# microsoft/esvit

Hardware: NVIDIA H100
Metric: multi-crop images/sec, Swin-T W7 pretrain step (2 global 224^2 + 8 local 96^2 crops, DDINOLoss V+R, K=65536) (higher is better)
Workload: dtype bf16

## Files before the change

### esvit_b200/csrc/window_attn.cu

```cuda
#include <cstdlib>

#include "wa_common.cuh"
#include "window_attn7.cuh"
#include "window_attn14.cuh"
#include "window_attn_probs.cuh"

namespace wa {

static bool make_geo(Geo& g, int B, int H, int W, int C, int nH, int ws, int shift) {
  if (B <= 0 || C != nH * HD || (ws != 7 && ws != 14) || shift < 0 || shift >= ws) return false;
  g.B = B; g.H = H; g.W = W; g.C = C; g.nH = nH; g.shift = shift;
  g.Hp = (H + ws - 1) / ws * ws;
  g.Wp = (W + ws - 1) / ws * ws;
  g.nWy = g.Hp / ws;
  g.nWx = g.Wp / ws;
  const char* d = getenv("ESVIT_ATTN_DBG");
  g.dbg = d ? atoi(d) : 0;
  return true;
}

static int windows_grid(int nwin, int nH, int per_sm) {
  int gy = esvit_num_sms() * per_sm / nH;
  if (gy < 1) gy = 1;
  const char* e = getenv("ESVIT_ATTN_GY");
  if (e && atoi(e) > 0) gy = atoi(e);
  return gy > nwin ? nwin : gy;
}

template <typename K>
static cudaError_t opt_in_smem(K kernel, size_t smem) {
  return smem > 48 * 1024 ? cudaFuncSetAttribute(kernel, cudaFuncAttributeMaxDynamicSharedMemorySize, (int)smem)
                          : cudaSuccess;
}

}

ESVIT_API int esvit_window_attn_expand_bias(const float* bias_table, float* bias_ws, int nH, int ws, void* stream) {
  if (nH <= 0 || (ws != 7 && ws != 14) || !bias_table) return ESVIT_ERR_BAD_ARG;
  if (ws == 7) {
    if (!bias_ws) return ESVIT_ERR_BAD_ARG;
    wa::expand_bias7_kernel<<<nH, 256, 0, (cudaStream_t)stream>>>(bias_table, bias_ws, nH);
  }
  ESVIT_LAUNCH_CHECK();
}

ESVIT_API int esvit_window_attn_fwd(const void* qkv, const void* qkv_bias, const float* bias_table, float* bias_ws,
                                    int bias_ready, void* out, float* lse, int B, int H, int W, int C, int nH, int ws,
                                    int shift, float scale, void* stream) {
  wa::Geo g;
  if (!wa::make_geo(g, B, H, W, C, nH, ws, shift)) return ESVIT_ERR_BAD_ARG;
  const int nwin = B * g.nWy * g.nWx;
  cudaStream_t st = (cudaStream_t)stream;
  const bf16* q = (const bf16*)qkv;
  const bf16* qb = (const bf16*)qkv_bias;
  if (ws == 7) {
    if (!bias_ws) return ESVIT_ERR_BAD_ARG;
    if (!bias_ready) wa::expand_bias7_kernel<<<nH, 256, 0, st>>>(bias_table, bias_ws, nH);
    const size_t smem = wa::fwd7_smem();
    const int gx = wa::windows_grid(nwin, nH, 16);
    if (shift > 0)
      wa::window_attn_fwd7_kernel<true><<<dim3(nH, gx), 128, smem, st>>>(q, qb, bias_ws, (bf16*)out, lse, g, scale, nwin);
    else
      wa::window_attn_fwd7_kernel<false><<<dim3(nH, gx), 128, smem, st>>>(q, qb, bias_ws, (bf16*)out, lse, g, scale, nwin);
  } else {
    const size_t smem = wa::fwd14_smem();
    cudaError_t e = wa::opt_in_smem(wa::window_attn_fwd14_kernel<true>, smem);
    if (e == cudaSuccess) e = wa::opt_in_smem(wa::window_attn_fwd14_kernel<false>, smem);
    if (e != cudaSuccess) return (int)e;
    const dim3 grid(nH, wa::windows_grid(nwin, nH, 2));
    if (shift > 0)
      wa::window_attn_fwd14_kernel<true><<<grid, wa::T14, smem, st>>>(q, qb, bias_table, (bf16*)out, lse, g, scale, nwin);
    else
      wa::window_attn_fwd14_kernel<false><<<grid, wa::T14, smem, st>>>(q, qb, bias_table, (bf16*)out, lse, g, scale, nwin);
  }
  ESVIT_LAUNCH_CHECK();
}

ESVIT_API int esvit_window_attn_bwd(const void* qkv, const void* qkv_bias, const float* bias_table, float* bias_ws,
                                    int bias_ready, const void* out, const void* dout, const float* lse, void* dqkv,
                                    float* dbias_table, float* dqkv_bias, int B, int H, int W, int C, int nH, int ws,
                                    int shift, float scale, void* stream) {
  wa::Geo g;
  if (!wa::make_geo(g, B, H, W, C, nH, ws, shift)) return ESVIT_ERR_BAD_ARG;
  const int nwin = B * g.nWy * g.nWx;
  cudaStream_t st = (cudaStream_t)stream;
  const bf16* q = (const bf16*)qkv;
  const bf16* qb = (const bf16*)qkv_bias;
  if (ws == 7) {
    if (!bias_ws) return ESVIT_ERR_BAD_ARG;
    if (!bias_ready) wa::expand_bias7_kernel<<<nH, 256, 0, st>>>(bias_table, bias_ws, nH);
    const size_t smem = wa::bwd7_smem();
    cudaError_t e = wa::opt_in_smem(wa::window_attn_bwd7_kernel<true>, smem);
    if (e == cudaSuccess) e = wa::opt_in_smem(wa::window_attn_bwd7_kernel<false>, smem);
    if (e != cudaSuccess) return (int)e;
    const int gx = wa::windows_grid(nwin, nH, 12);
    if (shift > 0)
      wa::window_attn_bwd7_kernel<true><<<dim3(nH, gx), 128, smem, st>>>(q, qb, bias_ws, (const bf16*)out,
                                                                         (const bf16*)dout, lse, (bf16*)dqkv,
                                                                         dbias_table, dqkv_bias, g, scale, nwin);
    else
      wa::window_attn_bwd7_kernel<false><<<dim3(nH, gx), 128, smem, st>>>(q, qb, bias_ws, (const bf16*)out,
                                                                          (const bf16*)dout, lse, (bf16*)dqkv,
                                                                          dbias_table, dqkv_bias, g, scale, nwin);
  } else {
    if (!bias_ws) return ESVIT_ERR_BAD_ARG;
    const size_t smem = wa::bwd14_smem();
    cudaError_t e = wa::opt_in_smem(wa::window_attn_bwd14_kernel<true>, smem);
    if (e == cudaSuccess) e = wa::opt_in_smem(wa::window_attn_bwd14_kernel<false>, smem);
    if (e == cudaSuccess) e = cudaMemsetAsync(bias_ws, 0, (size_t)nH * wa::GACC14 * sizeof(float), st);
    if (e != cudaSuccess) return (int)e;
    const dim3 grid(nH, wa::windows_grid(nwin, nH, 2));
    if (shift > 0)
      wa::window_attn_bwd14_kernel<true><<<grid, wa::T14, smem, st>>>(q, qb, bias_table, (const bf16*)out, (const bf16*)dout,
                                                                      lse, (bf16*)dqkv, bias_ws, dqkv_bias, g, scale, nwin);
    else
      wa::window_attn_bwd14_kernel<false><<<grid, wa::T14, smem, st>>>(q, qb, bias_table, (const bf16*)out, (const bf16*)dout,
                                                                       lse, (bf16*)dqkv, bias_ws, dqkv_bias, g, scale, nwin);
    wa::fold_dbias14_kernel<<<dim3(27, nH), 192, 0, st>>>(bias_ws, dbias_table, nH);
  }
  ESVIT_LAUNCH_CHECK();
}

ESVIT_API int esvit_window_attn_probs(const void* qkv, const void* qkv_bias, const float* bias_table, float* bias_ws,
                                      int bias_ready, float* probs, int B, int H, int W, int C, int nH, int ws,
                                      int shift, float scale, void* stream) {
  wa::Geo g;
  if (!wa::make_geo(g, B, H, W, C, nH, ws, shift) || !qkv || !qkv_bias || !bias_table || !probs) return ESVIT_ERR_BAD_ARG;
  const int nwin = B * g.nWy * g.nWx;
  cudaStream_t st = (cudaStream_t)stream;
  const bf16* q = (const bf16*)qkv;
  const bf16* qb = (const bf16*)qkv_bias;
  if (ws == 7) {
    if (!bias_ws) return ESVIT_ERR_BAD_ARG;
    if (!bias_ready) wa::expand_bias7_kernel<<<nH, 256, 0, st>>>(bias_table, bias_ws, nH);
    const size_t smem = wa::probs7_smem();
    const dim3 grid(nH, wa::windows_grid(nwin, nH, 16));
    if (shift > 0)
      wa::window_attn_probs7_kernel<true><<<grid, 128, smem, st>>>(q, qb, bias_ws, probs, g, scale, nwin);
    else
      wa::window_attn_probs7_kernel<false><<<grid, 128, smem, st>>>(q, qb, bias_ws, probs, g, scale, nwin);
  } else {
    const size_t smem = wa::probs14_smem();
    cudaError_t e = wa::opt_in_smem(wa::window_attn_probs14_kernel<true>, smem);
    if (e == cudaSuccess) e = wa::opt_in_smem(wa::window_attn_probs14_kernel<false>, smem);
    if (e != cudaSuccess) return (int)e;
    const dim3 grid(nH, wa::windows_grid(nwin, nH, 2));
    if (shift > 0)
      wa::window_attn_probs14_kernel<true><<<grid, wa::T14, smem, st>>>(q, qb, bias_table, probs, g, scale, nwin);
    else
      wa::window_attn_probs14_kernel<false><<<grid, wa::T14, smem, st>>>(q, qb, bias_table, probs, g, scale, nwin);
  }
  ESVIT_LAUNCH_CHECK();
}
```

### esvit_b200/csrc/window_attn7.cuh

```cuda
#pragma once
#include "wa_common.cuh"

namespace wa {

constexpr int BLD = 72;
constexpr int TILE7 = 64 * LD;

__global__ void __launch_bounds__(256) expand_bias7_kernel(const float* __restrict__ bias_table, float* __restrict__ bexp,
                                                           int nH) {
  const int h = blockIdx.x;
  for (int i = threadIdx.x; i < 64 * 64; i += blockDim.x) {
    const int row = i >> 6, col = i & 63;
    float v = -INFINITY;
    if (col < 49) v = row < 49 ? bias_table[bias_index<7>(row, col) * nH + h] * LOG2E : 0.f;
    bexp[(long long)h * 4096 + i] = v;
  }
}

template <bool BWD, int NTHREADS = 128, int NPART = 3>
__device__ __forceinline__ void issue7(const Geo& g, int win, int h, const bf16* __restrict__ qkv,
                                       const uint4 (&bchunk)[3], const bf16* __restrict__ dout,
                                       const bf16* __restrict__ out, const float* __restrict__ lse, bf16* tiles,
                                       float* Lraw, int* tok, int* rid) {
  constexpr int WS = 7, NT = 49;
  const int wx = win % g.nWx, wy = (win / g.nWx) % g.nWy, b = win / (g.nWx * g.nWy);
  const int c16 = threadIdx.x & 3;
#pragma unroll
  for (int kk = 0; kk < 256 / NTHREADS; kk++) {
    const int t = (threadIdx.x >> 2) + (NTHREADS / 4) * kk;
    int tk = -1, r = 0;
    if (t < NT) slot_info<WS>(g, b, wy, wx, t, tk, r);
    const bf16* src_row = qkv + (long long)(tk >= 0 ? tk : 0) * 3 * g.C + h * HD + c16 * 8;
    const int nbytes = (t < NT && g.dbg != 1) ? 16 : 0;
    if (t < NT && tk < 0) {
#pragma unroll
      for (int part = 0; part < NPART; part++)
        *reinterpret_cast<uint4*>(tiles + part * TILE7 + t * LD + c16 * 8) = bchunk[part];
    } else {
#pragma unroll
      for (int part = 0; part < NPART; part++)
        cp_async16(tiles + part * TILE7 + t * LD + c16 * 8, src_row + part * g.C, nbytes);
    }
    if (BWD) {
      const long long off = (long long)(tk >= 0 ? tk : 0) * g.C + h * HD + c16 * 8;
      const int nb = (tk >= 0 && g.dbg != 1) ? 16 : 0;
      cp_async16(tiles + 3 * TILE7 + t * LD + c16 * 8, dout + off, nb);
      cp_async16(tiles + 4 * TILE7 + t * LD + c16 * 8, out + off, nb);
    }
    if (c16 == 0) {
      tok[t] = tk;
      rid[t] = r;
      if (BWD) cp_async4(Lraw + t, lse + ((long long)win * g.nH + h) * NT + (t < NT ? t : 0), t < NT ? 4 : 0);
    }
  }
}

template <bool SHIFT>
__global__ void __launch_bounds__(128, 4) window_attn_fwd7_kernel(
    const bf16* __restrict__ qkv, const bf16* __restrict__ qkv_bias, const float* __restrict__ bexp,
    bf16* __restrict__ out, float* __restrict__ lse, Geo g, float scale, int nwin_total) {
  constexpr int WS = 7;
  using C = Cfg<WS>;
  static_assert(C::KP == 64 && C::NW == 4, "fast path assumes a 64-slot window and 4 warps");
  extern __shared__ __align__(16) unsigned char smraw[];
  bf16* tiles = reinterpret_cast<bf16*>(smraw);
  int* tokb = reinterpret_cast<int*>(tiles + 2 * 3 * TILE7);
  int* ridb = tokb + 2 * 64;

  const int h = blockIdx.x;
  const int lane = threadIdx.x & 31, warp = threadIdx.x >> 5;
  const int r0 = warp * 16, rA = r0 + (lane >> 2), rB = rA + 8;
  int win = blockIdx.y, stage = 0;
  uint4 bchunk[3];
#pragma unroll
  for (int part = 0; part < 3; part++)
    bchunk[part] = __ldg(reinterpret_cast<const uint4*>(qkv_bias + part * g.C + h * HD + (threadIdx.x & 3) * 8));
  if (win < nwin_total) issue7<false>(g, win, h, qkv, bchunk, nullptr, nullptr, nullptr, tiles, nullptr, tokb, ridb);
  cp_async_commit();

  float breg[C::NT8][4];
  {
    const float* bh = bexp + (long long)h * 4096 + (lane & 3) * 2;
#pragma unroll
    for (int nt = 0; nt < C::NT8; nt++) {
      const float2 a = __ldg(reinterpret_cast<const float2*>(bh + rA * 64 + nt * 8));
      const float2 b = __ldg(reinterpret_cast<const float2*>(bh + rB * 64 + nt * 8));
      breg[nt][0] = a.x; breg[nt][1] = a.y; breg[nt][2] = b.x; breg[nt][3] = b.y;
    }
  }
  const float c = scale * LOG2E;
  const int frag_off = (r0 + (lane & 7) + ((lane >> 3) & 1) * 8) * LD + (lane >> 4) * 8;

  for (; win < nwin_total; win += gridDim.y, stage ^= 1) {
    const int nxt = win + gridDim.y;
    if (nxt < nwin_total)
      issue7<false>(g, nxt, h, qkv, bchunk, nullptr, nullptr, nullptr, tiles + (stage ^ 1) * 3 * TILE7, nullptr,
                    tokb + (stage ^ 1) * 64, ridb + (stage ^ 1) * 64);
    cp_async_commit();
    cp_async_wait<1>();
    __syncthreads();
    const bf16* Qs = tiles + stage * 3 * TILE7;
    const bf16* Ks = Qs + TILE7;
    const bf16* Vs = Ks + TILE7;
    const int* tok = tokb + stage * 64;
    const int* rid = ridb + stage * 64;
    if (g.dbg == 2) { __syncthreads(); continue; }
    const int tA = rA < C::NT ? tok[rA] : -1, tB = rB < C::NT ? tok[rB] : -1;
    if (!__any_sync(0xffffffffu, tA >= 0 || tB >= 0)) {
      if ((lane & 3) == 0) {
        float* l = lse + ((long long)win * g.nH + h) * C::NT;
        if (rA < C::NT) l[rA] = 0.f;
        if (rB < C::NT) l[rB] = 0.f;
      }
      __syncthreads();
      continue;
    }

    uint32_t qa[2][4];
    ldsm_x4(qa[0], Qs + frag_off);
    ldsm_x4(qa[1], Qs + frag_off + 16);
    float acc[C::NT8][4];
    float m0 = -INFINITY, m1 = -INFINITY;
    int ridA = 0, ridB = 0;
    if (SHIFT) { ridA = rid[rA]; ridB = rid[rB]; }
#pragma unroll
    for (int nt = 0; nt < C::NT8; nt++) {
      acc[nt][0] = acc[nt][1] = acc[nt][2] = acc[nt][3] = 0.f;
      uint32_t kb[4];
      ldsm_x4(kb, Ks + (nt * 8 + (lane & 7)) * LD + (lane >> 3) * 8);
      mma16816(acc[nt], qa[0], kb[0], kb[1]);
      mma16816(acc[nt], qa[1], kb[2], kb[3]);
#pragma unroll
      for (int i = 0; i < 4; i++) acc[nt][i] = fmaf(acc[nt][i], c, breg[nt][i]);
      if (SHIFT) {
        const int2 rc = *reinterpret_cast<const int2*>(rid + nt * 8 + (lane & 3) * 2);
        if (ridA != rc.x) acc[nt][0] += -100.f * LOG2E;
        if (ridA != rc.y) acc[nt][1] += -100.f * LOG2E;
        if (ridB != rc.x) acc[nt][2] += -100.f * LOG2E;
        if (ridB != rc.y) acc[nt][3] += -100.f * LOG2E;
      }
      m0 = fmaxf(m0, fmaxf(acc[nt][0], acc[nt][1]));
      m1 = fmaxf(m1, fmaxf(acc[nt][2], acc[nt][3]));
    }
    m0 = fmaxf(m0, __shfl_xor_sync(0xffffffffu, m0, 1));
    m0 = fmaxf(m0, __shfl_xor_sync(0xffffffffu, m0, 2));
    m1 = fmaxf(m1, __shfl_xor_sync(0xffffffffu, m1, 1));
    m1 = fmaxf(m1, __shfl_xor_sync(0xffffffffu, m1, 2));
    float s0x = 0.f, s0y = 0.f, s1x = 0.f, s1y = 0.f;
#pragma unroll
    for (int nt = 0; nt < C::NT8; nt++) {
      acc[nt][0] = ex2(acc[nt][0] - m0);
      acc[nt][1] = ex2(acc[nt][1] - m0);
      acc[nt][2] = ex2(acc[nt][2] - m1);
      acc[nt][3] = ex2(acc[nt][3] - m1);
      s0x += acc[nt][0]; s0y += acc[nt][1];
      s1x += acc[nt][2]; s1y += acc[nt][3];
    }
    float s0 = s0x + s0y, s1 = s1x + s1y;
    s0 += __shfl_xor_sync(0xffffffffu, s0, 1);
    s0 += __shfl_xor_sync(0xffffffffu, s0, 2);
    s1 += __shfl_xor_sync(0xffffffffu, s1, 1);
    s1 += __shfl_xor_sync(0xffffffffu, s1, 2);
    const float i0 = __fdividef(1.f, s0), i1 = __fdividef(1.f, s1);
    if ((lane & 3) == 0) {
      float* l = lse + ((long long)win * g.nH + h) * C::NT;
      if (rA < C::NT) l[rA] = (m0 + lg2(s0)) * LN2;
      if (rB < C::NT) l[rB] = (m1 + lg2(s1)) * LN2;
    }
#pragma unroll
    for (int nt = 0; nt < C::NT8; nt++) {
      acc[nt][0] *= i0; acc[nt][1] *= i0;
      acc[nt][2] *= i1; acc[nt][3] *= i1;
    }
    float o[4][4];
#pragma unroll
    for (int dt = 0; dt < 4; dt++) o[dt][0] = o[dt][1] = o[dt][2] = o[dt][3] = 0.f;
#pragma unroll
    for (int kk = 0; kk < C::MT; kk++) {
      uint32_t pa[4];
      pa[0] = pack_bf162(acc[2 * kk][0], acc[2 * kk][1]);
      pa[1] = pack_bf162(acc[2 * kk][2], acc[2 * kk][3]);
      pa[2] = pack_bf162(acc[2 * kk + 1][0], acc[2 * kk + 1][1]);
      pa[3] = pack_bf162(acc[2 * kk + 1][2], acc[2 * kk + 1][3]);
      const bf16* vp = Vs + (kk * 16 + (lane & 7) + ((lane >> 3) & 1) * 8) * LD + (lane >> 4) * 8;
      uint32_t vb[4];
      ldsm_x4_t(vb, vp);
      mma16816(o[0], pa, vb[0], vb[1]);
      mma16816(o[1], pa, vb[2], vb[3]);
      ldsm_x4_t(vb, vp + 16);
      mma16816(o[2], pa, vb[0], vb[1]);
      mma16816(o[3], pa, vb[2], vb[3]);
    }
#pragma unroll
    for (int dt = 0; dt < 4; dt++) {
      const int d = h * HD + dt * 8 + (lane & 3) * 2;
      if (tA >= 0) *reinterpret_cast<uint32_t*>(out + (long long)tA * g.C + d) = pack_bf162(o[dt][0], o[dt][1]);
      if (tB >= 0) *reinterpret_cast<uint32_t*>(out + (long long)tB * g.C + d) = pack_bf162(o[dt][2], o[dt][3]);
    }
    __syncthreads();
  }
  cp_async_wait<0>();
}

static size_t fwd7_smem() { return (size_t)2 * 3 * TILE7 * 2 + (size_t)4 * 64 * 4; }

template <bool SHIFT>
__global__ void __launch_bounds__(128, 3) window_attn_bwd7_kernel(
    const bf16* __restrict__ qkv, const bf16* __restrict__ qkv_bias, const float* __restrict__ bexp,
    const bf16* __restrict__ out, const bf16* __restrict__ dout, const float* __restrict__ lse,
    bf16* __restrict__ dqkv, float* __restrict__ dbias_table, float* __restrict__ dqkv_bias, Geo g, float scale,
    int nwin_total) {
  constexpr int WS = 7;
  using C = Cfg<WS>;
  constexpr int NTHREADS = 128;
  static_assert(C::KP == 64 && C::NW == 4, "fast path assumes a 64-slot window and 4 tiles per phase");
  extern __shared__ __align__(16) unsigned char smraw[];
  bf16* tiles = reinterpret_cast<bf16*>(smraw);
  float* bm = reinterpret_cast<float*>(tiles + 2 * 5 * TILE7);
  float* dbt = bm + C::KP * BLD;
  float* dqb = dbt + C::NB + 1;
  float* Dsm = dqb + 3 * HD;
  float* Lrawb = Dsm + C::KP;
  int* tokb = reinterpret_cast<int*>(Lrawb + 2 * 64);
  int* ridb = tokb + 2 * 64;

  const int h = blockIdx.x;
  const int lane = threadIdx.x & 31, warp = threadIdx.x >> 5;
  int win = blockIdx.y, stage = 0;
  uint4 bchunk[3];
#pragma unroll
  for (int part = 0; part < 3; part++)
    bchunk[part] = __ldg(reinterpret_cast<const uint4*>(qkv_bias + part * g.C + h * HD + (threadIdx.x & 3) * 8));
  if (win < nwin_total) issue7<true, NTHREADS>(g, win, h, qkv, bchunk, dout, out, lse, tiles, Lrawb, tokb, ridb);
  cp_async_commit();

  for (int i = threadIdx.x; i < C::KP * C::KP / 4; i += NTHREADS) {
    const int row = i >> 4, c4 = (i & 15) * 4;
    float4 v = __ldg(reinterpret_cast<const float4*>(bexp + (long long)h * 4096 + row * 64 + c4));
    if (row >= C::NT) v = make_float4(-INFINITY, -INFINITY, -INFINITY, -INFINITY);
    *reinterpret_cast<float4*>(bm + row * BLD + c4) = v;
  }
  for (int i = threadIdx.x; i < C::NB; i += NTHREADS) dbt[i] = 0.f;
  for (int i = threadIdx.x; i < 3 * HD; i += NTHREADS) dqb[i] = 0.f;
  float dsacc[C::NT8][4];
#pragma unroll
  for (int nt = 0; nt < C::NT8; nt++) dsacc[nt][0] = dsacc[nt][1] = dsacc[nt][2] = dsacc[nt][3] = 0.f;

  const float c = scale * LOG2E;
  const int r0 = warp * 16;
  const int rA = r0 + (lane >> 2), rB = rA + 8;
  const int frag_off = (r0 + (lane & 7) + ((lane >> 3) & 1) * 8) * LD + (lane >> 4) * 8;

  for (; win < nwin_total; win += gridDim.y, stage ^= 1) {
    const int nxt = win + gridDim.y;
    if (nxt < nwin_total)
      issue7<true, NTHREADS>(g, nxt, h, qkv, bchunk, dout, out, lse, tiles + (stage ^ 1) * 5 * TILE7, Lrawb + (stage ^ 1) * 64,
                   tokb + (stage ^ 1) * 64, ridb + (stage ^ 1) * 64);
    cp_async_commit();
    cp_async_wait<1>();
    __syncthreads();
    const bf16* Qs = tiles + stage * 5 * TILE7;
    const bf16* Ks = Qs + TILE7;
    const bf16* Vs = Ks + TILE7;
    const bf16* dOs = Vs + TILE7;
    const bf16* Os = dOs + TILE7;
    const float* Lraw = Lrawb + stage * 64;
    const int* tok = tokb + stage * 64;
    const int* rid = ridb + stage * 64;
    if (g.dbg == 2) { __syncthreads(); continue; }
    {
      const int t = threadIdx.x >> 1, half = threadIdx.x & 1;
      float part = 0.f;
#pragma unroll
      for (int k = 0; k < 2; k++) {
        float fd[8], fo[8];
        unpack8(*reinterpret_cast<const bf16x8*>(dOs + t * LD + half * 16 + k * 8), fd);
        unpack8(*reinterpret_cast<const bf16x8*>(Os + t * LD + half * 16 + k * 8), fo);
#pragma unroll
        for (int j = 0; j < 8; j++) part += fd[j] * fo[j];
      }
      part += __shfl_xor_sync(0xffffffffu, part, 1);
      if (half == 0) Dsm[t] = part;
    }
    __syncthreads();

    const int tA = rA < C::NT ? tok[rA] : -1, tB = rB < C::NT ? tok[rB] : -1;
    int ridA = 0, ridB = 0;
    if (SHIFT) { ridA = rid[rA]; ridB = rid[rB]; }
    const unsigned b0 = __ballot_sync(0xffffffffu, tok[lane] >= 0), b1 = __ballot_sync(0xffffffffu, tok[lane + 32] >= 0);
    const unsigned qvalid = ((b0 & 0xffffu) ? 1u : 0u) | ((b0 >> 16) ? 2u : 0u) | ((b1 & 0xffffu) ? 4u : 0u) | ((b1 >> 16) ? 8u : 0u);
    if ((qvalid >> warp) & 1u) {
      uint32_t qa[2][4], da[2][4];
      ldsm_x4(qa[0], Qs + frag_off);
      ldsm_x4(qa[1], Qs + frag_off + 16);
      ldsm_x4(da[0], dOs + frag_off);
      ldsm_x4(da[1], dOs + frag_off + 16);
      const float lA = Lraw[rA] * LOG2E, lB = Lraw[rB] * LOG2E, DA = Dsm[rA], DB = Dsm[rB];
      float dq[4][4];
#pragma unroll
      for (int dt = 0; dt < 4; dt++) dq[dt][0] = dq[dt][1] = dq[dt][2] = dq[dt][3] = 0.f;
#pragma unroll
      for (int kk = 0; kk < 4; kk++) {
        float ds2[2][4];
#pragma unroll
        for (int hf = 0; hf < 2; hf++) {
          const int nt = 2 * kk + hf;
          float sacc[4] = {0.f, 0.f, 0.f, 0.f};
          ds2[hf][0] = ds2[hf][1] = ds2[hf][2] = ds2[hf][3] = 0.f;
          uint32_t kb[4];
          const int boff = (nt * 8 + (lane & 7)) * LD + (lane >> 3) * 8;
          ldsm_x4(kb, Ks + boff);
          mma16816(sacc, qa[0], kb[0], kb[1]);
          mma16816(sacc, qa[1], kb[2], kb[3]);
          ldsm_x4(kb, Vs + boff);
          mma16816(ds2[hf], da[0], kb[0], kb[1]);
          mma16816(ds2[hf], da[1], kb[2], kb[3]);
          const int c0 = nt * 8 + (lane & 3) * 2;
          const float2 bA = *reinterpret_cast<const float2*>(bm + rA * BLD + c0);
          const float2 bB = *reinterpret_cast<const float2*>(bm + rB * BLD + c0);
          float sv[4] = {fmaf(sacc[0], c, bA.x) - lA, fmaf(sacc[1], c, bA.y) - lA, fmaf(sacc[2], c, bB.x) - lB,
                         fmaf(sacc[3], c, bB.y) - lB};
          if (SHIFT) {
            const int2 rc = *reinterpret_cast<const int2*>(rid + c0);
            if (ridA != rc.x) sv[0] += -100.f * LOG2E;
            if (ridA != rc.y) sv[1] += -100.f * LOG2E;
            if (ridB != rc.x) sv[2] += -100.f * LOG2E;
            if (ridB != rc.y) sv[3] += -100.f * LOG2E;
          }
          ds2[hf][0] = ex2(sv[0]) * (ds2[hf][0] - DA);
          ds2[hf][1] = ex2(sv[1]) * (ds2[hf][1] - DA);
          ds2[hf][2] = ex2(sv[2]) * (ds2[hf][2] - DB);
          ds2[hf][3] = ex2(sv[3]) * (ds2[hf][3] - DB);
#pragma unroll
          for (int e = 0; e < 4; e++) dsacc[nt][e] += ds2[hf][e];
        }
        uint32_t sa[4];
        sa[0] = pack_bf162(ds2[0][0], ds2[0][1]);
        sa[1] = pack_bf162(ds2[0][2], ds2[0][3]);
        sa[2] = pack_bf162(ds2[1][0], ds2[1][1]);
        sa[3] = pack_bf162(ds2[1][2], ds2[1][3]);
        const bf16* kp = Ks + (kk * 16 + (lane & 7) + ((lane >> 3) & 1) * 8) * LD + (lane >> 4) * 8;
        uint32_t kb[4];
        ldsm_x4_t(kb, kp);
        mma16816(dq[0], sa, kb[0], kb[1]);
        mma16816(dq[1], sa, kb[2], kb[3]);
        ldsm_x4_t(kb, kp + 16);
        mma16816(dq[2], sa, kb[0], kb[1]);
        mma16816(dq[3], sa, kb[2], kb[3]);
      }
#pragma unroll
      for (int dt = 0; dt < 4; dt++) {
        const int d = h * HD + dt * 8 + (lane & 3) * 2;
        if (tA >= 0)
          *reinterpret_cast<uint32_t*>(dqkv + (long long)tA * 3 * g.C + d) = pack_bf162(dq[dt][0] * scale, dq[dt][1] * scale);
        if (tB >= 0)
          *reinterpret_cast<uint32_t*>(dqkv + (long long)tB * 3 * g.C + d) = pack_bf162(dq[dt][2] * scale, dq[dt][3] * scale);
      }
      colsum_to_smem(dq, scale, dqb, lane);
    }
    {
      uint32_t ka[2][4], va[2][4];
      ldsm_x4(ka[0], Ks + frag_off);
      ldsm_x4(ka[1], Ks + frag_off + 16);
      ldsm_x4(va[0], Vs + frag_off);
      ldsm_x4(va[1], Vs + frag_off + 16);
      float dv[4][4], dk[4][4];
#pragma unroll
      for (int dt = 0; dt < 4; dt++) {
        dv[dt][0] = dv[dt][1] = dv[dt][2] = dv[dt][3] = 0.f;
        dk[dt][0] = dk[dt][1] = dk[dt][2] = dk[dt][3] = 0.f;
      }
#pragma unroll
      for (int qq = 0; qq < 4; qq++) {
        if (!((qvalid >> qq) & 1u)) continue;
        float pT[2][4], dsT[2][4];
#pragma unroll
        for (int hf = 0; hf < 2; hf++) {
          const int nt = 2 * qq + hf;
          pT[hf][0] = pT[hf][1] = pT[hf][2] = pT[hf][3] = 0.f;
          dsT[hf][0] = dsT[hf][1] = dsT[hf][2] = dsT[hf][3] = 0.f;
          uint32_t qb[4];
          const int boff = (nt * 8 + (lane & 7)) * LD + (lane >> 3) * 8;
          ldsm_x4(qb, Qs + boff);
          mma16816(pT[hf], ka[0], qb[0], qb[1]);
          mma16816(pT[hf], ka[1], qb[2], qb[3]);
          ldsm_x4(qb, dOs + boff);
          mma16816(dsT[hf], va[0], qb[0], qb[1]);
          mma16816(dsT[hf], va[1], qb[2], qb[3]);
          const int q0 = nt * 8 + (lane & 3) * 2;
          const float2 lq = *reinterpret_cast<const float2*>(Lraw + q0);
          const float2 Dq = *reinterpret_cast<const float2*>(Dsm + q0);
          float sv[4] = {fmaf(pT[hf][0], c, bm[q0 * BLD + rA]) - lq.x * LOG2E,
                         fmaf(pT[hf][1], c, bm[(q0 + 1) * BLD + rA]) - lq.y * LOG2E,
                         fmaf(pT[hf][2], c, bm[q0 * BLD + rB]) - lq.x * LOG2E,
                         fmaf(pT[hf][3], c, bm[(q0 + 1) * BLD + rB]) - lq.y * LOG2E};
          if (SHIFT) {
            const int2 rq = *reinterpret_cast<const int2*>(rid + q0);
            if (ridA != rq.x) sv[0] += -100.f * LOG2E;
            if (ridA != rq.y) sv[1] += -100.f * LOG2E;
            if (ridB != rq.x) sv[2] += -100.f * LOG2E;
            if (ridB != rq.y) sv[3] += -100.f * LOG2E;
          }
          pT[hf][0] = ex2(sv[0]); pT[hf][1] = ex2(sv[1]); pT[hf][2] = ex2(sv[2]); pT[hf][3] = ex2(sv[3]);
          dsT[hf][0] = pT[hf][0] * (dsT[hf][0] - Dq.x);
          dsT[hf][1] = pT[hf][1] * (dsT[hf][1] - Dq.y);
          dsT[hf][2] = pT[hf][2] * (dsT[hf][2] - Dq.x);
          dsT[hf][3] = pT[hf][3] * (dsT[hf][3] - Dq.y);
        }
        uint32_t pa[4], sa[4];
        pa[0] = pack_bf162(pT[0][0], pT[0][1]);
        pa[1] = pack_bf162(pT[0][2], pT[0][3]);
        pa[2] = pack_bf162(pT[1][0], pT[1][1]);
        pa[3] = pack_bf162(pT[1][2], pT[1][3]);
        sa[0] = pack_bf162(dsT[0][0], dsT[0][1]);
        sa[1] = pack_bf162(dsT[0][2], dsT[0][3]);
        sa[2] = pack_bf162(dsT[1][0], dsT[1][1]);
        sa[3] = pack_bf162(dsT[1][2], dsT[1][3]);
        const int toff = (qq * 16 + (lane & 7) + ((lane >> 3) & 1) * 8) * LD + (lane >> 4) * 8;
        uint32_t bb[4];
        ldsm_x4_t(bb, dOs + toff);
        mma16816(dv[0], pa, bb[0], bb[1]);
        mma16816(dv[1], pa, bb[2], bb[3]);
        ldsm_x4_t(bb, dOs + toff + 16);
        mma16816(dv[2], pa, bb[0], bb[1]);
        mma16816(dv[3], pa, bb[2], bb[3]);
        ldsm_x4_t(bb, Qs + toff);
        mma16816(dk[0], sa, bb[0], bb[1]);
        mma16816(dk[1], sa, bb[2], bb[3]);
        ldsm_x4_t(bb, Qs + toff + 16);
        mma16816(dk[2], sa, bb[0], bb[1]);
        mma16816(dk[3], sa, bb[2], bb[3]);
      }
#pragma unroll
      for (int dt = 0; dt < 4; dt++) {
        const int d = h * HD + dt * 8 + (lane & 3) * 2;
        if (tA >= 0) {
          bf16* base = dqkv + (long long)tA * 3 * g.C + d;
          *reinterpret_cast<uint32_t*>(base + g.C) = pack_bf162(dk[dt][0] * scale, dk[dt][1] * scale);
          *reinterpret_cast<uint32_t*>(base + 2 * g.C) = pack_bf162(dv[dt][0], dv[dt][1]);
        }
        if (tB >= 0) {
          bf16* base = dqkv + (long long)tB * 3 * g.C + d;
          *reinterpret_cast<uint32_t*>(base + g.C) = pack_bf162(dk[dt][2] * scale, dk[dt][3] * scale);
          *reinterpret_cast<uint32_t*>(base + 2 * g.C) = pack_bf162(dv[dt][2], dv[dt][3]);
        }
      }
      colsum_to_smem(dk, scale, dqb + HD, lane);
      colsum_to_smem(dv, 1.f, dqb + 2 * HD, lane);
    }
    __syncthreads();
  }
  cp_async_wait<0>();
#pragma unroll
  for (int nt = 0; nt < C::NT8; nt++)
#pragma unroll
    for (int e = 0; e < 4; e++) {
      const int row = (e < 2) ? rA : rB;
      const int col = nt * 8 + (lane & 3) * 2 + (e & 1);
      if (row < C::NT && col < C::NT) atomicAdd(&dbt[bias_index<WS>(row, col)], dsacc[nt][e]);
    }
  __syncthreads();
  for (int i = threadIdx.x; i < C::NB; i += NTHREADS) atomicAdd(&dbias_table[i * g.nH + h], dbt[i]);
  for (int i = threadIdx.x; i < 3 * HD; i += NTHREADS)
    atomicAdd(&dqkv_bias[(i / HD) * g.C + h * HD + (i % HD)], dqb[i]);
}

static size_t bwd7_smem() {
  using C = Cfg<7>;
  return (size_t)2 * 5 * TILE7 * 2 + (size_t)(C::KP * BLD + C::NB + 1 + 3 * HD + C::KP + 2 * 64) * 4 + (size_t)4 * 64 * 4;
}

}
```

Before: 1242.

## Reuse P and dS via shared memory in window-7 attention backward instead of recomputing

The window-7 backward kernel now writes the softmax probabilities P and dS once to shared bf16 tiles and reads them transposed with ldmatrix for the dK/dV pass. This removes the second QK^T and dO·V^T recompute. The bias is held in registers instead of a shared float matrix, and the D = rowsum(dO·O) reduction moves into each warp, removing a block barrier. Outputs are staged through shared memory so they are written as coalesced 16-byte rows. The dK/dV column sums now accumulate in registers across windows, and the grid per SM drops from 12 to 3, which reduces parallelism and adds smem traffic and extra syncs.

```diff
diff --git a/esvit_b200/csrc/window_attn.cu b/esvit_b200/csrc/window_attn.cu
--- a/esvit_b200/csrc/window_attn.cu
+++ b/esvit_b200/csrc/window_attn.cu
@@ -93,7 +93,7 @@
     cudaError_t e = wa::opt_in_smem(wa::window_attn_bwd7_kernel<true>, smem);
     if (e == cudaSuccess) e = wa::opt_in_smem(wa::window_attn_bwd7_kernel<false>, smem);
     if (e != cudaSuccess) return (int)e;
-    const int gx = wa::windows_grid(nwin, nH, 12);
+    const int gx = wa::windows_grid(nwin, nH, 3);
     if (shift > 0)
       wa::window_attn_bwd7_kernel<true><<<dim3(nH, gx), 128, smem, st>>>(q, qb, bias_ws, (const bf16*)out,
                                                                          (const bf16*)dout, lse, (bf16*)dqkv,
diff --git a/esvit_b200/csrc/window_attn7.cuh b/esvit_b200/csrc/window_attn7.cuh
--- a/esvit_b200/csrc/window_attn7.cuh
+++ b/esvit_b200/csrc/window_attn7.cuh
@@ -3,7 +3,6 @@
 
 namespace wa {
 
-constexpr int BLD = 72;
 constexpr int TILE7 = 64 * LD;
 
 __global__ void __launch_bounds__(256) expand_bias7_kernel(const float* __restrict__ bias_table, float* __restrict__ bexp,
@@ -204,6 +203,34 @@
 
 static size_t fwd7_smem() { return (size_t)2 * 3 * TILE7 * 2 + (size_t)4 * 64 * 4; }
 
+constexpr int PLD = 72;
+
+__device__ __forceinline__ void store_rows7(const float (&t)[4][4], float scale, bf16* stg, const int* tok,
+                                            bf16* __restrict__ dst, long long ld, int lane) {
+  const int rr = lane >> 2, c16 = lane & 3;
+  __syncwarp();
+#pragma unroll
+  for (int dt = 0; dt < 4; dt++) {
+    *reinterpret_cast<uint32_t*>(stg + rr * LD + dt * 8 + c16 * 2) = pack_bf162(t[dt][0] * scale, t[dt][1] * scale);
+    *reinterpret_cast<uint32_t*>(stg + (rr + 8) * LD + dt * 8 + c16 * 2) = pack_bf162(t[dt][2] * scale, t[dt][3] * scale);
+  }
+  __syncwarp();
+#pragma unroll
+  for (int i = 0; i < 2; i++) {
+    const int row = rr + 8 * i, tk = tok[row];
+    if (tk >= 0)
+      *reinterpret_cast<uint4*>(dst + tk * ld + c16 * 8) = *reinterpret_cast<const uint4*>(stg + row * LD + c16 * 8);
+  }
+}
+
+__device__ __forceinline__ void colsum_acc(const float (&t)[4][4], float (&cs)[4][2]) {
+#pragma unroll
+  for (int dt = 0; dt < 4; dt++) {
+    cs[dt][0] += t[dt][0] + t[dt][2];
+    cs[dt][1] += t[dt][1] + t[dt][3];
+  }
+}
+
 template <bool SHIFT>
 __global__ void __launch_bounds__(128, 3) window_attn_bwd7_kernel(
     const bf16* __restrict__ qkv, const bf16* __restrict__ qkv_bias, const float* __restrict__ bexp,
@@ -216,11 +243,11 @@
   static_assert(C::KP == 64 && C::NW == 4, "fast path assumes a 64-slot window and 4 tiles per phase");
   extern __shared__ __align__(16) unsigned char smraw[];
   bf16* tiles = reinterpret_cast<bf16*>(smraw);
-  float* bm = reinterpret_cast<float*>(tiles + 2 * 5 * TILE7);
-  float* dbt = bm + C::KP * BLD;
+  bf16* Ps = tiles + 2 * 5 * TILE7;
+  bf16* dSs = Ps + C::KP * PLD;
+  float* dbt = reinterpret_cast<float*>(dSs + C::KP * PLD);
   float* dqb = dbt + C::NB + 1;
-  float* Dsm = dqb + 3 * HD;
-  float* Lrawb = Dsm + C::KP;
+  float* Lrawb = dqb + 3 * HD;
   int* tokb = reinterpret_cast<int*>(Lrawb + 2 * 64);
   int* ridb = tokb + 2 * 64;
 
@@ -231,116 +258,123 @@
 #pragma unroll
   for (int part = 0; part < 3; part++)
     bchunk[part] = __ldg(reinterpret_cast<const uint4*>(qkv_bias + part * g.C + h * HD + (threadIdx.x & 3) * 8));
-  if (win < nwin_total) issue7<true, NTHREADS>(g, win, h, qkv, bchunk, dout, out, lse, tiles, Lrawb, tokb, ridb);
+  auto issue = [&](int w, int st) {
+    issue7<true, NTHREADS>(g, w, h, qkv, bchunk, dout, out, lse, tiles + st * 5 * TILE7, Lrawb + st * 64, tokb + st * 64,
+                           ridb + st * 64);
+  };
+  if (win < nwin_total) issue(win, 0);
   cp_async_commit();
 
-  for (int i = threadIdx.x; i < C::KP * C::KP / 4; i += NTHREADS) {
-    const int row = i >> 4, c4 = (i & 15) * 4;
-    float4 v = __ldg(reinterpret_cast<const float4*>(bexp + (long long)h * 4096 + row * 64 + c4));
-    if (row >= C::NT) v = make_float4(-INFINITY, -INFINITY, -INFINITY, -INFINITY);
-    *reinterpret_cast<float4*>(bm + row * BLD + c4) = v;
-  }
   for (int i = threadIdx.x; i < C::NB; i += NTHREADS) dbt[i] = 0.f;
   for (int i = threadIdx.x; i < 3 * HD; i += NTHREADS) dqb[i] = 0.f;
-  float dsacc[C::NT8][4];
-#pragma unroll
-  for (int nt = 0; nt < C::NT8; nt++) dsacc[nt][0] = dsacc[nt][1] = dsacc[nt][2] = dsacc[nt][3] = 0.f;
 
   const float c = scale * LOG2E;
   const int r0 = warp * 16;
   const int rA = r0 + (lane >> 2), rB = rA + 8;
   const int frag_off = (r0 + (lane & 7) + ((lane >> 3) & 1) * 8) * LD + (lane >> 4) * 8;
+  float breg[C::NT8][4];
+  {
+    const float* bh = bexp + (long long)h * 4096 + (lane & 3) * 2;
+#pragma unroll
+    for (int nt = 0; nt < C::NT8; nt++) {
+      const float2 a = __ldg(reinterpret_cast<const float2*>(bh + rA * 64 + nt * 8));
+      const float2 b = __ldg(reinterpret_cast<const float2*>(bh + rB * 64 + nt * 8));
+      breg[nt][0] = rA < C::NT ? a.x : -INFINITY; breg[nt][1] = rA < C::NT ? a.y : -INFINITY;
+      breg[nt][2] = rB < C::NT ? b.x : -INFINITY; breg[nt][3] = rB < C::NT ? b.y : -INFINITY;
+    }
+  }
+  float dsacc[C::NT8][4];
+#pragma unroll
+  for (int nt = 0; nt < C::NT8; nt++) dsacc[nt][0] = dsacc[nt][1] = dsacc[nt][2] = dsacc[nt][3] = 0.f;
+  float csk[4][2] = {}, csv[4][2] = {};
 
   for (; win < nwin_total; win += gridDim.y, stage ^= 1) {
+    cp_async_wait<0>();
+    __syncthreads();
     const int nxt = win + gridDim.y;
-    if (nxt < nwin_total)
-      issue7<true, NTHREADS>(g, nxt, h, qkv, bchunk, dout, out, lse, tiles + (stage ^ 1) * 5 * TILE7, Lrawb + (stage ^ 1) * 64,
-                   tokb + (stage ^ 1) * 64, ridb + (stage ^ 1) * 64);
+    if (nxt < nwin_total) issue(nxt, stage ^ 1);
     cp_async_commit();
-    cp_async_wait<1>();
-    __syncthreads();
     const bf16* Qs = tiles + stage * 5 * TILE7;
     const bf16* Ks = Qs + TILE7;
     const bf16* Vs = Ks + TILE7;
     const bf16* dOs = Vs + TILE7;
-    const bf16* Os = dOs + TILE7;
+    bf16* Os = tiles + stage * 5 * TILE7 + 4 * TILE7;
+    bf16* stg = Os + r0 * LD;
     const float* Lraw = Lrawb + stage * 64;
     const int* tok = tokb + stage * 64;
     const int* rid = ridb + stage * 64;
-    if (g.dbg == 2) { __syncthreads(); continue; }
-    {
-      const int t = threadIdx.x >> 1, half = threadIdx.x & 1;
-      float part = 0.f;
-#pragma unroll
-      for (int k = 0; k < 2; k++) {
-        float fd[8], fo[8];
-        unpack8(*reinterpret_cast<const bf16x8*>(dOs + t * LD + half * 16 + k * 8), fd);
-        unpack8(*reinterpret_cast<const bf16x8*>(Os + t * LD + half * 16 + k * 8), fo);
-#pragma unroll
-        for (int j = 0; j < 8; j++) part += fd[j] * fo[j];
-      }
-      part += __shfl_xor_sync(0xffffffffu, part, 1);
-      if (half == 0) Dsm[t] = part;
-    }
-    __syncthreads();
-
-    const int tA = rA < C::NT ? tok[rA] : -1, tB = rB < C::NT ? tok[rB] : -1;
-    int ridA = 0, ridB = 0;
-    if (SHIFT) { ridA = rid[rA]; ridB = rid[rB]; }
+    if (g.dbg == 2) continue;
+
     const unsigned b0 = __ballot_sync(0xffffffffu, tok[lane] >= 0), b1 = __ballot_sync(0xffffffffu, tok[lane + 32] >= 0);
     const unsigned qvalid = ((b0 & 0xffffu) ? 1u : 0u) | ((b0 >> 16) ? 2u : 0u) | ((b1 & 0xffffu) ? 4u : 0u) | ((b1 >> 16) ? 8u : 0u);
     if ((qvalid >> warp) & 1u) {
+      float DA = 0.f, DB = 0.f;
+      {
+        float fd[8], fo[8];
+        unpack8(*reinterpret_cast<const bf16x8*>(dOs + rA * LD + (lane & 3) * 8), fd);
+        unpack8(*reinterpret_cast<const bf16x8*>(Os + rA * LD + (lane & 3) * 8), fo);
+#pragma unroll
+        for (int j = 0; j < 8; j++) DA += fd[j] * fo[j];
+        unpack8(*reinterpret_cast<const bf16x8*>(dOs + rB * LD + (lane & 3) * 8), fd);
+        unpack8(*reinterpret_cast<const bf16x8*>(Os + rB * LD + (lane & 3) * 8), fo);
+#pragma unroll
+        for (int j = 0; j < 8; j++) DB += fd[j] * fo[j];
+        DA += __shfl_xor_sync(0xffffffffu, DA, 1);
+        DA += __shfl_xor_sync(0xffffffffu, DA, 2);
+        DB += __shfl_xor_sync(0xffffffffu, DB, 1);
+        DB += __shfl_xor_sync(0xffffffffu, DB, 2);
+      }
       uint32_t qa[2][4], da[2][4];
       ldsm_x4(qa[0], Qs + frag_off);
       ldsm_x4(qa[1], Qs + frag_off + 16);
       ldsm_x4(da[0], dOs + frag_off);
       ldsm_x4(da[1], dOs + frag_off + 16);
-      const float lA = Lraw[rA] * LOG2E, lB = Lraw[rB] * LOG2E, DA = Dsm[rA], DB = Dsm[rB];
+      const float lA = Lraw[rA] * LOG2E, lB = Lraw[rB] * LOG2E;
+      int ridA = 0, ridB = 0;
+      if (SHIFT) { ridA = rid[rA]; ridB = rid[rB]; }
+#pragma unroll
+      for (int nt = 0; nt < C::NT8; nt++) {
+        float sacc[4] = {0.f, 0.f, 0.f, 0.f}, ds[4] = {0.f, 0.f, 0.f, 0.f};
+        uint32_t kb[4];
+        const int boff = (nt * 8 + (lane & 7)) * LD + (lane >> 3) * 8;
+        ldsm_x4(kb, Ks + boff);
+        mma16816(sacc, qa[0], kb[0], kb[1]);
+        mma16816(sacc, qa[1], kb[2], kb[3]);
+        ldsm_x4(kb, Vs + boff);
+        mma16816(ds, da[0], kb[0], kb[1]);
+        mma16816(ds, da[1], kb[2], kb[3]);
+        float sv[4] = {fmaf(sacc[0], c, breg[nt][0]) - lA, fmaf(sacc[1], c, breg[nt][1]) - lA,
+                       fmaf(sacc[2], c, breg[nt][2]) - lB, fmaf(sacc[3], c, breg[nt][3]) - lB};
+        const int c0 = nt * 8 + (lane & 3) * 2;
+        if (SHIFT) {
+          const int2 rc = *reinterpret_cast<const int2*>(rid + c0);
+          if (ridA != rc.x) sv[0] += -100.f * LOG2E;
+          if (ridA != rc.y) sv[1] += -100.f * LOG2E;
+          if (ridB != rc.x) sv[2] += -100.f * LOG2E;
+          if (ridB != rc.y) sv[3] += -100.f * LOG2E;
+        }
+        const float p[4] = {ex2(sv[0]), ex2(sv[1]), ex2(sv[2]), ex2(sv[3])};
+        ds[0] = p[0] * (ds[0] - DA);
+        ds[1] = p[1] * (ds[1] - DA);
+        ds[2] = p[2] * (ds[2] - DB);
+        ds[3] = p[3] * (ds[3] - DB);
+#pragma unroll
+        for (int e = 0; e < 4; e++) dsacc[nt][e] += ds[e];
+        *reinterpret_cast<uint32_t*>(Ps + rA * PLD + c0) = pack_bf162(p[0], p[1]);
+        *reinterpret_cast<uint32_t*>(Ps + rB * PLD + c0) = pack_bf162(p[2], p[3]);
+        *reinterpret_cast<uint32_t*>(dSs + rA * PLD + c0) = pack_bf162(ds[0], ds[1]);
+        *reinterpret_cast<uint32_t*>(dSs + rB * PLD + c0) = pack_bf162(ds[2], ds[3]);
+      }
+      __syncwarp();
       float dq[4][4];
 #pragma unroll
       for (int dt = 0; dt < 4; dt++) dq[dt][0] = dq[dt][1] = dq[dt][2] = dq[dt][3] = 0.f;
+      const int soff = (r0 + (lane & 7) + ((lane >> 3) & 1) * 8) * PLD + (lane >> 4) * 8;
 #pragma unroll
       for (int kk = 0; kk < 4; kk++) {
-        float ds2[2][4];
-#pragma unroll
-        for (int hf = 0; hf < 2; hf++) {
-          const int nt = 2 * kk + hf;
-          float sacc[4] = {0.f, 0.f, 0.f, 0.f};
-          ds2[hf][0] = ds2[hf][1] = ds2[hf][2] = ds2[hf][3] = 0.f;
-          uint32_t kb[4];
-          const int boff = (nt * 8 + (lane & 7)) * LD + (lane >> 3) * 8;
-          ldsm_x4(kb, Ks + boff);
-          mma16816(sacc, qa[0], kb[0], kb[1]);
-          mma16816(sacc, qa[1], kb[2], kb[3]);
-          ldsm_x4(kb, Vs + boff);
-          mma16816(ds2[hf], da[0], kb[0], kb[1]);
-          mma16816(ds2[hf], da[1], kb[2], kb[3]);
-          const int c0 = nt * 8 + (lane & 3) * 2;
-          const float2 bA = *reinterpret_cast<const float2*>(bm + rA * BLD + c0);
-          const float2 bB = *reinterpret_cast<const float2*>(bm + rB * BLD + c0);
-          float sv[4] = {fmaf(sacc[0], c, bA.x) - lA, fmaf(sacc[1], c, bA.y) - lA, fmaf(sacc[2], c, bB.x) - lB,
-                         fmaf(sacc[3], c, bB.y) - lB};
-          if (SHIFT) {
-            const int2 rc = *reinterpret_cast<const int2*>(rid + c0);
-            if (ridA != rc.x) sv[0] += -100.f * LOG2E;
-            if (ridA != rc.y) sv[1] += -100.f * LOG2E;
-            if (ridB != rc.x) sv[2] += -100.f * LOG2E;
-            if (ridB != rc.y) sv[3] += -100.f * LOG2E;
-          }
-          ds2[hf][0] = ex2(sv[0]) * (ds2[hf][0] - DA);
-          ds2[hf][1] = ex2(sv[1]) * (ds2[hf][1] - DA);
-          ds2[hf][2] = ex2(sv[2]) * (ds2[hf][2] - DB);
-          ds2[hf][3] = ex2(sv[3]) * (ds2[hf][3] - DB);
-#pragma unroll
-          for (int e = 0; e < 4; e++) dsacc[nt][e] += ds2[hf][e];
-        }
-        uint32_t sa[4];
-        sa[0] = pack_bf162(ds2[0][0], ds2[0][1]);
-        sa[1] = pack_bf162(ds2[0][2], ds2[0][3]);
-        sa[2] = pack_bf162(ds2[1][0], ds2[1][1]);
-        sa[3] = pack_bf162(ds2[1][2], ds2[1][3]);
+        uint32_t sa[4], kb[4];
+        ldsm_x4(sa, dSs + soff + kk * 16);
         const bf16* kp = Ks + (kk * 16 + (lane & 7) + ((lane >> 3) & 1) * 8) * LD + (lane >> 4) * 8;
-        uint32_t kb[4];
         ldsm_x4_t(kb, kp);
         mma16816(dq[0], sa, kb[0], kb[1]);
         mma16816(dq[1], sa, kb[2], kb[3]);
@@ -348,74 +382,24 @@
         mma16816(dq[2], sa, kb[0], kb[1]);
         mma16816(dq[3], sa, kb[2], kb[3]);
       }
-#pragma unroll
-      for (int dt = 0; dt < 4; dt++) {
-        const int d = h * HD + dt * 8 + (lane & 3) * 2;
-        if (tA >= 0)
-          *reinterpret_cast<uint32_t*>(dqkv + (long long)tA * 3 * g.C + d) = pack_bf162(dq[dt][0] * scale, dq[dt][1] * scale);
-        if (tB >= 0)
-          *reinterpret_cast<uint32_t*>(dqkv + (long long)tB * 3 * g.C + d) = pack_bf162(dq[dt][2] * scale, dq[dt][3] * scale);
-      }
+      store_rows7(dq, scale, stg, tok + r0, dqkv + h * HD, 3LL * g.C, lane);
       colsum_to_smem(dq, scale, dqb, lane);
     }
+    __syncthreads();
     {
-      uint32_t ka[2][4], va[2][4];
-      ldsm_x4(ka[0], Ks + frag_off);
-      ldsm_x4(ka[1], Ks + frag_off + 16);
-      ldsm_x4(va[0], Vs + frag_off);
-      ldsm_x4(va[1], Vs + frag_off + 16);
       float dv[4][4], dk[4][4];
 #pragma unroll
       for (int dt = 0; dt < 4; dt++) {
         dv[dt][0] = dv[dt][1] = dv[dt][2] = dv[dt][3] = 0.f;
         dk[dt][0] = dk[dt][1] = dk[dt][2] = dk[dt][3] = 0.f;
       }
+      const int aoff = ((lane >> 4) * 8 + (lane & 7)) * PLD + r0 + ((lane >> 3) & 1) * 8;
 #pragma unroll
       for (int qq = 0; qq < 4; qq++) {
         if (!((qvalid >> qq) & 1u)) continue;
-        float pT[2][4], dsT[2][4];
-#pragma unroll
-        for (int hf = 0; hf < 2; hf++) {
-          const int nt = 2 * qq + hf;
-          pT[hf][0] = pT[hf][1] = pT[hf][2] = pT[hf][3] = 0.f;
-          dsT[hf][0] = dsT[hf][1] = dsT[hf][2] = dsT[hf][3] = 0.f;
-          uint32_t qb[4];
-          const int boff = (nt * 8 + (lane & 7)) * LD + (lane >> 3) * 8;
-          ldsm_x4(qb, Qs + boff);
-          mma16816(pT[hf], ka[0], qb[0], qb[1]);
-          mma16816(pT[hf], ka[1], qb[2], qb[3]);
-          ldsm_x4(qb, dOs + boff);
-          mma16816(dsT[hf], va[0], qb[0], qb[1]);
-          mma16816(dsT[hf], va[1], qb[2], qb[3]);
-          const int q0 = nt * 8 + (lane & 3) * 2;
-          const float2 lq = *reinterpret_cast<const float2*>(Lraw + q0);
-          const float2 Dq = *reinterpret_cast<const float2*>(Dsm + q0);
-          float sv[4] = {fmaf(pT[hf][0], c, bm[q0 * BLD + rA]) - lq.x * LOG2E,
-                         fmaf(pT[hf][1], c, bm[(q0 + 1) * BLD + rA]) - lq.y * LOG2E,
-                         fmaf(pT[hf][2], c, bm[q0 * BLD + rB]) - lq.x * LOG2E,
-                         fmaf(pT[hf][3], c, bm[(q0 + 1) * BLD + rB]) - lq.y * LOG2E};
-          if (SHIFT) {
-            const int2 rq = *reinterpret_cast<const int2*>(rid + q0);
-            if (ridA != rq.x) sv[0] += -100.f * LOG2E;
-            if (ridA != rq.y) sv[1] += -100.f * LOG2E;
-            if (ridB != rq.x) sv[2] += -100.f * LOG2E;
-            if (ridB != rq.y) sv[3] += -100.f * LOG2E;
-          }
-          pT[hf][0] = ex2(sv[0]); pT[hf][1] = ex2(sv[1]); pT[hf][2] = ex2(sv[2]); pT[hf][3] = ex2(sv[3]);
-          dsT[hf][0] = pT[hf][0] * (dsT[hf][0] - Dq.x);
-          dsT[hf][1] = pT[hf][1] * (dsT[hf][1] - Dq.y);
-          dsT[hf][2] = pT[hf][2] * (dsT[hf][2] - Dq.x);
-          dsT[hf][3] = pT[hf][3] * (dsT[hf][3] - Dq.y);
-        }
         uint32_t pa[4], sa[4];
-        pa[0] = pack_bf162(pT[0][0], pT[0][1]);
-        pa[1] = pack_bf162(pT[0][2], pT[0][3]);
-        pa[2] = pack_bf162(pT[1][0], pT[1][1]);
-        pa[3] = pack_bf162(pT[1][2], pT[1][3]);
-        sa[0] = pack_bf162(dsT[0][0], dsT[0][1]);
-        sa[1] = pack_bf162(dsT[0][2], dsT[0][3]);
-        sa[2] = pack_bf162(dsT[1][0], dsT[1][1]);
-        sa[3] = pack_bf162(dsT[1][2], dsT[1][3]);
+        ldsm_x4_t(pa, Ps + qq * 16 * PLD + aoff);
+        ldsm_x4_t(sa, dSs + qq * 16 * PLD + aoff);
         const int toff = (qq * 16 + (lane & 7) + ((lane >> 3) & 1) * 8) * LD + (lane >> 4) * 8;
         uint32_t bb[4];
         ldsm_x4_t(bb, dOs + toff);
@@ -431,24 +415,11 @@
         mma16816(dk[2], sa, bb[0], bb[1]);
         mma16816(dk[3], sa, bb[2], bb[3]);
       }
-#pragma unroll
-      for (int dt = 0; dt < 4; dt++) {
-        const int d = h * HD + dt * 8 + (lane & 3) * 2;
-        if (tA >= 0) {
-          bf16* base = dqkv + (long long)tA * 3 * g.C + d;
-          *reinterpret_cast<uint32_t*>(base + g.C) = pack_bf162(dk[dt][0] * scale, dk[dt][1] * scale);
-          *reinterpret_cast<uint32_t*>(base + 2 * g.C) = pack_bf162(dv[dt][0], dv[dt][1]);
-        }
-        if (tB >= 0) {
-          bf16* base = dqkv + (long long)tB * 3 * g.C + d;
-          *reinterpret_cast<uint32_t*>(base + g.C) = pack_bf162(dk[dt][2] * scale, dk[dt][3] * scale);
-          *reinterpret_cast<uint32_t*>(base + 2 * g.C) = pack_bf162(dv[dt][2], dv[dt][3]);
-        }
-      }
-      colsum_to_smem(dk, scale, dqb + HD, lane);
-      colsum_to_smem(dv, 1.f, dqb + 2 * HD, lane);
-    }
-    __syncthreads();
+      store_rows7(dk, scale, stg, tok + r0, dqkv + g.C + h * HD, 3LL * g.C, lane);
+      store_rows7(dv, 1.f, stg, tok + r0, dqkv + 2 * g.C + h * HD, 3LL * g.C, lane);
+      colsum_acc(dk, csk);
+      colsum_acc(dv, csv);
+    }
   }
   cp_async_wait<0>();
 #pragma unroll
@@ -459,6 +430,22 @@
       const int col = nt * 8 + (lane & 3) * 2 + (e & 1);
       if (row < C::NT && col < C::NT) atomicAdd(&dbt[bias_index<WS>(row, col)], dsacc[nt][e]);
     }
+#pragma unroll
+  for (int dt = 0; dt < 4; dt++)
+#pragma unroll
+    for (int e = 0; e < 2; e++) {
+      float k = csk[dt][e] * scale, v = csv[dt][e];
+#pragma unroll
+      for (int o = 4; o < 32; o <<= 1) {
+        k += __shfl_xor_sync(0xffffffffu, k, o);
+        v += __shfl_xor_sync(0xffffffffu, v, o);
+      }
+      if (lane < 4) {
+        const int col = dt * 8 + lane * 2 + e;
+        atomicAdd(&dqb[HD + col], k);
+        atomicAdd(&dqb[2 * HD + col], v);
+      }
+    }
   __syncthreads();
   for (int i = threadIdx.x; i < C::NB; i += NTHREADS) atomicAdd(&dbias_table[i * g.nH + h], dbt[i]);
   for (int i = threadIdx.x; i < 3 * HD; i += NTHREADS)
@@ -467,7 +454,8 @@
 
 static size_t bwd7_smem() {
   using C = Cfg<7>;
-  return (size_t)2 * 5 * TILE7 * 2 + (size_t)(C::KP * BLD + C::NB + 1 + 3 * HD + C::KP + 2 * 64) * 4 + (size_t)4 * 64 * 4;
-}
-
-}
+  return (size_t)2 * 5 * TILE7 * 2 + (size_t)2 * C::KP * PLD * 2 + (size_t)(C::NB + 1 + 3 * HD + 2 * 64) * 4 +
+         (size_t)4 * 64 * 4;
+}
+
+}
```

Result: faster. 1294, median of 6 (+4.2%).
